# fcogidi/X3D-tf

Hardware: AMD Instinct MI355X
Metric: clips/sec (fwd+bwd) X3D-M 16x224^2; depthwise HBM GB/s (higher is better)
Workload: dtype bf16

## Files before the change

### x3d-tf_amd/csrc/pw_gemm_bf16.h

```cpp
#pragma once
#include <stdlib.h>

#include "pw_gemm.h"

typedef __attribute__((ext_vector_type(4))) short s16x4;
typedef __attribute__((ext_vector_type(8))) short s16x8;

#define PWB_BN 128
#define PWB_KCH 64
#define PWB_XP (PWB_BN + 32)
#define PWB_OP (PWB_BN + 4)

template <typename H, int VEC, int MT, int PRO, int EPI, int STRIDED, int OVEC, bool RAG = false>
__global__ __launch_bounds__(256) void pw_gemm_bf16_kernel(const PwGemmArgs a) {
  typedef typename HV<H>::x8 hx8; typedef typename HV<H>::x4 hx4; typedef typename HV<H>::x2 hx2;
  extern __shared__ __attribute__((aligned(16))) unsigned char smem_raw[];
  typedef H T;
  constexpr int BM = MT * 32, BN = PWB_BN, XP = PWB_XP, OP = PWB_OP, KCH = PWB_KCH;
  constexpr bool HAS_SUMS = (EPI == EPI_STATS) || (EPI == X3D_EPI_SWISH_BWD);
  constexpr bool BSTORE = (OVEC == 8);
  typedef __attribute__((ext_vector_type(4))) unsigned int u32x4_;
  constexpr int VPR = BN / VEC;
  constexpr int NSV = (KCH * VPR + 255) / 256;
  constexpr int ROWS_PT = BM / 16;
  constexpr int SLAB = (MT <= 2) ? MT : 1, NSLAB = MT / SLAB, ROWS_SL = 2 * SLAB;
  const int Kp = a.KC;
  const int WP = Kp + 8;
  constexpr size_t XO_BYTES = ((size_t)KCH * XP * 2 > (size_t)SLAB * 32 * OP * 4) ? (size_t)KCH * XP * 2 : (size_t)SLAB * 32 * OP * 4;
  H* Xs = (H*)smem_raw;
  float* Os = (float*)smem_raw;
  H* Ws = (H*)(smem_raw + XO_BYTES);
  float* Cs = (float*)(smem_raw + XO_BYTES + (size_t)BM * (a.KC + 8) * 2);

  const int tid = threadIdx.x, lane = tid & 63, wid = tid >> 6;
  const int r = lane & 31, half = lane >> 5;
  const int m0 = blockIdx.y * BM;
  const int tiles_per_n = (int)((a.P + BN - 1) / BN);
  const int total_tiles = tiles_per_n * a.N;
  const int tile_begin = blockIdx.x * a.tiles_per_block;
  const int tile_end = min(tile_begin + a.tiles_per_block, total_tiles);
  const int nkc = (Kp + KCH - 1) / KCH;

  if (a.wp) {
    const hx8* src = (const hx8*)((const H*)a.wp + (long long)m0 * WP);
    const int nvec = BM * WP / 8;
    const int lim = max(0, min(BM, a.wp_rows - m0)) * WP / 8;
    hx8 zero;
#pragma unroll
    for (int e = 0; e < 8; e++) zero[e] = (H)0.f;
#pragma unroll 4
    for (int i = tid; i < nvec; i += 256) ((hx8*)Ws)[i] = i < lim ? src[i] : zero;
  } else {
    const int wv = a.wvec;
    if (a.wsk == 1) {
      const int kv = Kp / wv;
      for (int i = tid; i < BM * kv; i += 256) {
        const int m = i / kv, k = (i - m * kv) * wv;
        const int gm = m0 + m;
        const float* src = a.w + (long long)gm * a.wsm + k;
        H* dst = &Ws[m * WP + k];
        for (int e = 0; e < wv; e += 1) dst[e] = (H)0.f;
        if (gm < a.M && k < a.K) {
          if (wv == 4) { const f32x4 v = *(const f32x4*)src; dst[0] = (H)v[0]; dst[1] = (H)v[1]; dst[2] = (H)v[2]; dst[3] = (H)v[3]; }
          else if (wv == 2) { const float2 v = *(const float2*)src; dst[0] = (H)v.x; dst[1] = (H)v.y; }
          else dst[0] = (H)src[0];
        }
      }
    } else {
      const int mv = BM / wv;
      for (int i = tid; i < Kp * mv; i += 256) {
        const int k = i / mv, m = (i - k * mv) * wv;
        const int gm = m0 + m;
        const float* src = a.w + (long long)k * a.wsk + gm;
        float v[4] = {0.f, 0.f, 0.f, 0.f};
        if (k < a.K) {
          if (wv == 4 && gm + 3 < a.M) { const f32x4 t = *(const f32x4*)src; v[0] = t[0]; v[1] = t[1]; v[2] = t[2]; v[3] = t[3]; }
          else for (int e = 0; e < wv; e++) if (gm + e < a.M) v[e] = src[e];
        }
        for (int e = 0; e < wv; e++) Ws[(m + e) * WP + k] = (H)v[e];
      }
    }
  }

  constexpr bool AFF = (PRO == PRO_AFFINE) || (PRO == PRO_AFFST);
  constexpr int CSW = AFF ? 2 : 4;
  const bool use_cs = AFF || a.K < 320;
  auto fill_coef = [&](int n) {
    if (!use_cs) return;
    if constexpr (PRO != PRO_NONE) {
      for (int k = tid; k < Kp; k += 256) {
        f32x4 c = {0.f, 0.f, 0.f, 0.f};
        if (k < a.K) {
          if constexpr (AFF) {
            const float g = a.gate ? a.gate[(long long)n * a.K + k] : 1.0f;
            c[0] = a.coef[k * 2] * g;
            c[1] = a.coef[k * 2 + 1] * g;
          } else if constexpr (PRO == PRO_TAIL) {
            c[0] = a.coef[k * 2]; c[1] = a.coef2 ? a.coef2[k * 2] : 1.0f;
            c[2] = a.coef[k * 2 + 1] + (a.coef2 ? a.coef2[k * 2 + 1] : 0.f);
          } else {
            c[0] = a.coef[k * 4]; c[1] = a.coef[k * 4 + 1]; c[2] = a.coef[k * 4 + 2];
          }
        }
        if constexpr (CSW == 2) *(float2*)&Cs[k * 2] = make_float2(c[0], c[1]);
        else *(f32x4*)&Cs[k * 4] = c;
      }
    }
  };
  if (tile_begin < tile_end) fill_coef(tile_begin / tiles_per_n);

  constexpr bool TWO = (PRO == PRO_BNBWD) || (PRO == PRO_TAIL);
  hx8 xr[NSV], yr[(TWO || STRIDED) ? NSV : 1];
  float xs1[(VEC == 1) ? NSV : 1], ys1[(VEC == 1 && TWO) ? NSV : 1];
  auto issue_loads = [&](int tile, int kc_idx) {
    const int n = tile / tiles_per_n;
    const long long p0 = (long long)(tile - n * tiles_per_n) * BN;
    const int k0 = kc_idx * KCH;
    const int kc = min(KCH, Kp - k0);
#pragma unroll
    for (int i = 0; i < NSV; i++) {
      const int v = tid + i * 256;
      const int k = v / VPR, pv = v - k * VPR;
      const int gk = k0 + k;
      const long long p = p0 + (long long)pv * VEC;
      const bool ok = (k < kc) && (gk < a.K) && (p < a.P);
      if constexpr (VEC == 8) {
        hx8 z;
#pragma unroll
        for (int e = 0; e < 8; e++) z[e] = (H)0.f;
        xr[i] = z;
        if constexpr (TWO) yr[i] = z;
        if constexpr (STRIDED) yr[i] = z;
        if (ok) {
          if constexpr (STRIDED) {
            strided_gather16<STRIDED>((const T*)a.x + ((long long)n * a.K + gk) * a.Pin, p, a.H, a.W, a.Ho, a.Wo, xr[i], yr[i],
                                      RAG ? (int)min((long long)8, a.P - p) : 8);
          } else {
            const long long o = ((long long)n * a.K + k0 + (tid >> 4)) * a.Pin + p0 + (tid & 15) * 8 + (long long)i * 16 * a.Pin;
            const long long left = RAG ? a.P - p : 8;
            if (left >= 8) {
              xr[i] = *(const hx8*)((const T*)a.x + o);
              if constexpr (TWO) yr[i] = *(const hx8*)((const T*)a.x2 + o);
            } else {
              xr[i] = load8_ragged<T, hx8>((const T*)a.x + o, (int)left);
              if constexpr (TWO) yr[i] = load8_ragged<T, hx8>((const T*)a.x2 + o, (int)left);
            }
          }
        }
      } else {
        xs1[i] = 0.f;
        if constexpr (TWO) ys1[i] = 0.f;
        if (ok) {
          long long src = p;
          if constexpr (STRIDED) {
            const int hw = a.Ho * a.Wo;
            const int t = (int)p / hw;
            const int rem = (int)p - t * hw;
            const int ho = rem / a.Wo, wo = rem - ho * a.Wo;
            src = ((long long)t * a.H + (long long)ho * a.stride) * a.W + (long long)wo * a.stride;
          }
          const long long o = ((long long)n * a.K + gk) * a.Pin + src;
          xs1[i] = to_f<T>(((const T*)a.x)[o]);
          if constexpr (TWO) ys1[i] = to_f<T>(((const T*)a.x2)[o]);
        }
      }
    }
  };
  auto commit = [&](int tile, int kc_idx) {
    const int n = tile / tiles_per_n;
    const int k0 = kc_idx * KCH;
    const int kc = min(KCH, Kp - k0);
#pragma unroll
    for (int i = 0; i < NSV; i++) {
      const int v = tid + i * 256;
      const int k = v / VPR, pv = v - k * VPR;
      if (k >= kc) continue;
      const int gk = k0 + k;
      H* dst = &Xs[k * XP + pv * VEC];
      if constexpr (PRO == PRO_NONE) {
        if constexpr (VEC == 8 && STRIDED) {
          hx8 o;
#pragma unroll
          for (int e = 0; e < 4; e++) { o[e] = xr[i][2 * e]; o[4 + e] = yr[i][2 * e]; }
          *(hx8*)dst = o;
        } else if constexpr (VEC == 8) *(hx8*)dst = xr[i];
        else dst[0] = (H)xs1[i];
      } else {
        float val[VEC];
        if constexpr (VEC == 8) {
#pragma unroll
          for (int e = 0; e < 8; e++) val[e] = (float)xr[i][e];
        } else {
          val[0] = xs1[i];
        }
        f32x4 cf;
        if (use_cs) {
          if constexpr (CSW == 2) { const float2 t2 = *(const float2*)&Cs[gk * 2]; cf[0] = t2.x; cf[1] = t2.y; cf[2] = 0.f; cf[3] = 0.f; }
          else cf = *(const f32x4*)&Cs[gk * 4];
        } else {
          const bool inb = gk < a.K;
          cf[3] = 0.f;
          if constexpr (AFF) {
            const float g = (inb && a.gate) ? a.gate[(long long)n * a.K + gk] : 1.0f;
            cf[0] = inb ? a.coef[gk * 2] * g : 0.f; cf[1] = inb ? a.coef[gk * 2 + 1] * g : 0.f; cf[2] = 0.f;
          } else if constexpr (PRO == PRO_TAIL) {
            cf[0] = inb ? a.coef[gk * 2] : 0.f; cf[1] = (inb && a.coef2) ? a.coef2[gk * 2] : (inb ? 1.0f : 0.f);
            cf[2] = inb ? a.coef[gk * 2 + 1] + (a.coef2 ? a.coef2[gk * 2 + 1] : 0.f) : 0.f;
          } else {
            cf[0] = inb ? a.coef[gk * 4] : 0.f; cf[1] = inb ? a.coef[gk * 4 + 1] : 0.f; cf[2] = inb ? a.coef[gk * 4 + 2] : 0.f;
          }
        }
        if constexpr (AFF) {
#pragma unroll
          for (int e = 0; e < VEC; e++) val[e] = cf[0] * val[e] + cf[1];
          act_vec<VEC>(val, a.act);
        } else {
#pragma unroll
          for (int e = 0; e < VEC; e++) {
            const float y2 = (VEC == 8) ? (float)yr[i][e] : ys1[i];
            val[e] = cf[0] * val[e] + cf[1] * y2 + cf[2];
            if constexpr (PRO == PRO_TAIL) val[e] = fmaxf(val[e], 0.f);
          }
        }
        VecIO<H, VEC>::store(dst, val);
        if constexpr (PRO == PRO_TAIL || PRO == PRO_AFFST) {
          const int n_ = tile / tiles_per_n;
          const long long p_ = (long long)(tile - n_ * tiles_per_n) * BN + (long long)pv * VEC;
          if (blockIdx.y == 0 && gk < a.K && p_ < a.P) {
            T* yd = (T*)a.ystore + ((long long)n_ * a.K + gk) * a.Pin + p_;
            if constexpr (VEC == 8) {
              if (!RAG || a.P - p_ >= 8) VecIO<T, 8>::store(yd, val);
              else for (int e = 0; e < (int)(a.P - p_); e++) yd[e] = from_f<T>(val[e]);
            } else {
              yd[0] = from_f<T>(val[0]);
            }
          }
        }
      }
    }
  };

  float st1[HAS_SUMS ? ROWS_PT : 1], st2[HAS_SUMS ? ROWS_PT : 1];
  if constexpr (HAS_SUMS) {
#pragma unroll
    for (int i = 0; i < ROWS_PT; i++) { st1[i] = 0.f; st2[i] = 0.f; }
  }

  const int g16 = lane >> 4, q = (lane & 15) >> 2, pp = lane & 3;
  const int tr_col = wid * 32 + 16 * (g16 & 1) + 4 * pp;
  const int tr_row = 8 * (g16 >> 1) + q;
  typedef s16x4 __attribute__((address_space(3))) * lds_s16x4_ptr;

  f32x16 acc[MT];
  if (tile_begin < tile_end) issue_loads(tile_begin, 0);
  if constexpr (BSTORE) {
    __amdgpu_buffer_rsrc_t r0 = __builtin_amdgcn_make_buffer_rsrc((T*)a.y, 0, 0, 0x00020000);
    u32x4_ z0 = {0u, 0u, 0u, 0u};
#pragma unroll
    for (int i = 0; i < ROWS_PT; i++) __builtin_amdgcn_raw_buffer_store_b128(z0, r0, 0x80000000u, 0, 0);
  }

  auto flush_sums = [&](int n) {
    if constexpr (HAS_SUMS) {
#pragma unroll
      for (int i = 0; i < ROWS_PT; i++) {
        float s1 = st1[i], s2 = st2[i];
        s1 = row16_sum(s1);
        s2 = row16_sum(s2);
        const int m = m0 + (tid >> 4) + 16 * i;
        if ((tid & 15) == 0 && m < a.M) {
          if constexpr (EPI == EPI_STATS) {
            if (a.stats) {
              double* sp = stats_replica(a.stats, a.M, blockIdx.x);
              atomic_add_d(&sp[m * 2], (double)s1);
              atomic_add_d(&sp[m * 2 + 1], (double)s2);
            }
          } else {
            double* d = a.nc_sums + ((long long)n * a.M + m) * 2;
            atomic_add_d(d, (double)s1);
            atomic_add_d(d + 1, (double)s2);
          }
        }
        st1[i] = 0.f;
        st2[i] = 0.f;
      }
    }
  };

  float bna_s[EPI == EPI_BNADD ? ROWS_PT : 1], bna_t[EPI == EPI_BNADD ? ROWS_PT : 1], bna_g[EPI == EPI_BNADD ? ROWS_PT : 1];
  if constexpr (EPI == EPI_BNADD) {
#pragma unroll
    for (int i = 0; i < ROWS_PT; i++) {
      const int m = m0 + (tid >> 4) + 16 * i;
      bnadd_coef(a, m, m < a.M, bna_s[i], bna_t[i], bna_g[i]);
    }
  }

  int n_prev = tile_begin < tile_end ? tile_begin / tiles_per_n : 0;
  for (int tile = tile_begin; tile < tile_end; ++tile) {
    const int n = tile / tiles_per_n;
    const long long p0 = (long long)(tile - n * tiles_per_n) * BN;
    if constexpr (EPI == X3D_EPI_SWISH_BWD) {
      if (n != n_prev) flush_sums(n_prev);
    }
    if constexpr (AFF) {
      if (n != n_prev && a.gate) fill_coef(n);
    }
    n_prev = n;
#pragma unroll
    for (int s = 0; s < MT; s++)
#pragma unroll
      for (int j = 0; j < 16; j++) acc[s][j] = 0.f;

    for (int kc_idx = 0; kc_idx < nkc; ++kc_idx) {
      const int k0 = kc_idx * KCH;
      const int kc = min(KCH, Kp - k0);
      __syncthreads();
      commit(tile, kc_idx);
      __syncthreads();
      if (kc_idx + 1 < nkc) issue_loads(tile, kc_idx + 1);
      else if (tile + 1 < tile_end) issue_loads(tile + 1, 0);
      for (int kk = 0; kk < kc; kk += 16) {
        const s16x4 b0 = __builtin_amdgcn_ds_read_tr16_b64_v4i16((lds_s16x4_ptr)(&Xs[(kk + tr_row) * XP + tr_col]));
        const s16x4 b1 = __builtin_amdgcn_ds_read_tr16_b64_v4i16((lds_s16x4_ptr)(&Xs[(kk + tr_row + 4) * XP + tr_col]));
        const s16x8 bs = {b0[0], b0[1], b0[2], b0[3], b1[0], b1[1], b1[2], b1[3]};
        const hx8 bfrag = __builtin_bit_cast(hx8, bs);
#pragma unroll
        for (int s = 0; s < MT; s++) {
          const hx8 afrag = *(const hx8*)&Ws[(s * 32 + r) * WP + k0 + kk + 8 * half];
          acc[s] = mfma16<H>(afrag, bfrag, acc[s]);
        }
      }
    }

    const int oc = (tid & 15) * 8;
    __amdgpu_buffer_rsrc_t yrsrc;
    if constexpr (BSTORE)
      yrsrc = __builtin_amdgcn_make_buffer_rsrc((T*)a.y + (long long)n * a.M * a.P, 0, (int)((long long)a.M * a.P * 2), 0x00020000);
    constexpr bool BNA_ = (EPI == EPI_BNADD);
    constexpr bool EPL8 = (OVEC == 8) && (EPI == X3D_EPI_ADD || EPI == X3D_EPI_SWISH_BWD || BNA_);
    constexpr bool EPL4 = (OVEC == 8) && (EPI == X3D_EPI_ADD_STRIDED);
    hx8 epl8[EPL8 ? ROWS_PT : 1];
    hx4 epl4[EPL4 ? ROWS_PT : 1];
    const int egv = !EPL4 ? 0 : ((a.eW & 7) == 0 ? 8 : ((a.eW & 3) == 0 ? 4 : ((a.eW & 1) == 0 ? 2 : 0)));
    const bool epl4_vec = egv != 0;
    constexpr bool SWB_ = (EPI == X3D_EPI_SWISH_BWD);
    float esb[(SWB_ || BNA_) ? ROWS_PT : 1], etb[(SWB_ || BNA_) ? ROWS_PT : 1], egt[(SWB_ || BNA_) ? ROWS_PT : 1];
    if constexpr (BNA_) {
#pragma unroll
      for (int i = 0; i < ROWS_PT; i++) { esb[i] = bna_s[i]; etb[i] = bna_t[i]; egt[i] = bna_g[i]; }
    }
    if constexpr (SWB_) {
#pragma unroll
      for (int i = 0; i < ROWS_PT; i++) {
        const int m = m0 + (tid >> 4) + 16 * i;
        const bool ok = m < a.M;
        esb[i] = ok ? a.b_ss[m * 2] : 0.f;
        etb[i] = ok ? a.b_ss[m * 2 + 1] : 0.f;
        egt[i] = (ok && a.egate) ? a.egate[(long long)n * a.M + m] : 1.0f;
      }
    }
    if constexpr (EPL8 || EPL4) {
#pragma unroll
      for (int i = 0; i < ROWS_PT; i++) {
        const int m = m0 + (tid >> 4) + 16 * i;
        const long long p = p0 + oc;
        if constexpr (EPL8) {
#pragma unroll
          for (int e = 0; e < 8; e++) epl8[i][e] = (H)0.f;
          if (m < a.M && p < a.P && (!BNA_ || a.add)) {
            const long long o = ((long long)n * a.M + m) * a.P + p;
            const T* src = (const T*)(EPI == X3D_EPI_SWISH_BWD ? a.braw : a.add) + o;
            if (!RAG || a.P - p >= 8) epl8[i] = *(const hx8*)src;
            else epl8[i] = load8_ragged<T, hx8>(src, (int)(a.P - p));
          }
        } else {
#pragma unroll
          for (int e = 0; e < 4; e++) epl4[i][e] = (H)0.f;
          if (epl4_vec && m < a.M && p < a.P) {
            const int hw = a.eH * a.eW;
            const int Hh = (a.eH + 1) >> 1, Wh = (a.eW + 1) >> 1;
            const int T_ = (int)a.P / hw;
            const T* abase = (const T*)a.add + ((long long)n * a.M + m) * T_ * Hh * Wh;
            if (egv == 8) {
              const int t = (int)p / hw;
              const int rem = (int)p - t * hw;
              const int h = rem / a.eW, w = rem - h * a.eW;
              if ((h & 1) == 0) epl4[i] = *(const hx4*)(abase + ((long long)t * Hh + (h >> 1)) * Wh + (w >> 1));
            } else if (egv == 4) {
#pragma unroll
              for (int gq = 0; gq < 2; gq++) {
                const int pe = (int)p + 4 * gq;
                if (RAG && pe >= (int)a.P) continue;
                const int t = pe / hw;
                const int rem = pe - t * hw;
                const int h = rem / a.eW, w = rem - h * a.eW;
                if ((h & 1) == 0) {
                  const hx2 v2 = *(const hx2*)(abase + ((long long)t * Hh + (h >> 1)) * Wh + (w >> 1));
                  epl4[i][2 * gq] = v2[0]; epl4[i][2 * gq + 1] = v2[1];
                }
              }
            } else {
#pragma unroll
              for (int gq = 0; gq < 4; gq++) {
                const int pe = (int)p + 2 * gq;
                if (RAG && pe >= (int)a.P) continue;
                const int t = pe / hw;
                const int rem = pe - t * hw;
                const int h = rem / a.eW, w = rem - h * a.eW;
                if ((h & 1) == 0) epl4[i][gq] = abase[((long long)t * Hh + (h >> 1)) * Wh + (w >> 1)];
              }
            }
          }
        }
      }
    }
#pragma unroll
    for (int sl = 0; sl < NSLAB; sl++) {
    __syncthreads();
#pragma unroll
    for (int s = 0; s < SLAB; s++)
#pragma unroll
      for (int j = 0; j < 16; j++)
        Os[(s * 32 + (j & 3) + 8 * (j >> 2) + 4 * half) * OP + wid * 32 + r] = acc[sl * SLAB + s][j];
    __syncthreads();
#pragma unroll
    for (int ii = 0; ii < ROWS_SL; ii++) {
      const int i = sl * ROWS_SL + ii;
      const int row = (tid >> 4) + 16 * ii;
      const int m = m0 + sl * SLAB * 32 + row;
      const long long p = p0 + oc;
      const bool rvalid = (m < a.M) && (p < a.P);
      if constexpr (!BSTORE) { if (!rvalid) continue; }
      float val[8];
      {
        const f32x4 v0 = *(const f32x4*)&Os[row * OP + oc], v1 = *(const f32x4*)&Os[row * OP + oc + 4];
#pragma unroll
        for (int e = 0; e < 4; e++) { val[e] = v0[e]; val[4 + e] = v1[e]; }
      }
      const long long o = ((long long)n * a.M + m) * a.P + p;
      const int nvalid = (OVEC == 8 && !RAG) ? 8 : (int)min((long long)8, a.P - p);
      if constexpr (EPI == X3D_EPI_ADD) {
        if constexpr (OVEC == 8) {
#pragma unroll
          for (int e = 0; e < 8; e++) val[e] += (float)epl8[i][e];
        } else {
          for (int e = 0; e < nvalid; e++) val[e] += to_f<T>(((const T*)a.add)[o + e]);
        }
      } else if constexpr (BNA_) {
        float ad[8];
        if constexpr (OVEC == 8) {
#pragma unroll
          for (int e = 0; e < 8; e++) ad[e] = (float)epl8[i][e];
        } else {
          for (int e = 0; e < 8; e++) ad[e] = (e < nvalid && a.add) ? to_f<T>(((const T*)a.add)[o + e]) : 0.f;
        }
        const float lo = a.eact == X3D_ACT_RELU ? 0.f : -__builtin_inff();
#pragma unroll
        for (int e = 0; e < 8; e++) val[e] = fmaxf(esb[i] * val[e] + etb[i] + egt[i] * ad[e], lo);
      } else if constexpr (EPI == X3D_EPI_ADD_STRIDED) {
        const int hw = a.eH * a.eW;
        const int Hh = (a.eH + 1) >> 1, Wh = (a.eW + 1) >> 1;
        const int T_ = (int)a.P / hw;
        if (epl4_vec) {
          if constexpr (EPL4) {
#pragma unroll
            for (int e = 0; e < 4; e++) val[2 * e] += (float)epl4[i][e];
          }
        } else if (m < a.M)
        for (int e = 0; e < nvalid; e++) {
          const int pe = (int)p + e;
          const int t = pe / hw;
          const int rem = pe - t * hw;
          const int h = rem / a.eW, w = rem - h * a.eW;
          if (((h | w) & 1) == 0) {
            const long long oa = ((((long long)n * a.M + m) * T_ + t) * Hh + (h >> 1)) * Wh + (w >> 1);
            val[e] += to_f<T>(((const T*)a.add)[oa]);
          }
        }
      } else if constexpr (EPI == X3D_EPI_SWISH_BWD) {
        float b[8];
        if constexpr (OVEC == 8) {
#pragma unroll
          for (int e = 0; e < 8; e++) b[e] = (float)epl8[i][e];
        } else {
          for (int e = 0; e < 8; e++) b[e] = (e < nvalid) ? to_f<T>(((const T*)a.braw)[o + e]) : 0.f;
        }
        const SwishCoef sc_ = swish_coef(esb[i], etb[i], egt[i]);
#pragma unroll
        for (int e = 0; e < 8; e++) {
          float xh_, d_;
          swish_bwd_(sc_, b[e], xh_, d_);
          const float dv = val[e] * d_;
          val[e] = dv;
          if (e < nvalid && rvalid) {
            st1[i] += dv;
            st2[i] += dv * b[e];
          }
        }
      }
      if constexpr (EPI == EPI_STATS) {
#pragma unroll
        for (int e = 0; e < 8; e++) {
          if (e < nvalid && rvalid) {
            st1[i] += val[e];
            st2[i] += val[e] * val[e];
          }
        }
      }
      if constexpr (BSTORE) {
        hx8 ov;
#pragma unroll
        for (int e = 0; e < 8; e++) ov[e] = (H)val[e];
        const unsigned off = (rvalid && (!RAG || nvalid == 8)) ? (unsigned)(((long long)m * a.P + p) * 2) : 0x80000000u;
        __builtin_amdgcn_raw_buffer_store_b128(__builtin_bit_cast(u32x4_, ov), yrsrc, off, 0, 0);
        if constexpr (RAG) {
          if (rvalid && nvalid < 8) store8_ragged<T, hx8>((T*)a.y + o, ov, nvalid);
        }
      } else if constexpr (OVEC == 8) {
        if (!RAG || nvalid == 8) VecIO<T, 8>::store((T*)a.y + o, val);
        else {
          for (int e = 0; e < nvalid; e++) ((T*)a.y)[o + e] = from_f<T>(val[e]);
        }
      } else {
        for (int e = 0; e < nvalid; e++) ((T*)a.y)[o + e] = from_f<T>(val[e]);
      }
    }
    }
  }

  if (tile_begin < tile_end) flush_sums(n_prev);
}

static inline size_t pw_bf16_lds_bytes(int mt, int K) {
  const int slab = mt <= 2 ? mt : 1;
  const size_t xb = (size_t)PWB_KCH * PWB_XP * 2, ob = (size_t)slab * 32 * PWB_OP * 4;
  return (xb > ob ? xb : ob) + (size_t)mt * 32 * (((K + 15) & ~15) + 8) * 2 + (K < 320 ? (size_t)((K + 15) & ~15) * 16 : (size_t)((K + 15) & ~15) * 8);
}

static inline int pw_bf16_pick_mt(int M, int K) {
  const int mt = ceil_div(M, 32);
#ifdef X3D_EXPERIMENTS
  const char* map = getenv("X3D_PW_MTMAP");
#else
  const char* map = nullptr;
#endif
  if (map) {
    for (const char* q = map; *q;) {
      const int key = atoi(q);
      const char* c = strchr(q, ':');
      if (!c) break;
      const int val = atoi(c + 1);
      if (key == mt && (val == 1 || val == 2 || val == 3 || val == 4 || val == 7) && pw_bf16_lds_bytes(val, K) <= 160 * 1024) return val;
      const char* n = strchr(c, ',');
      if (!n) break;
      q = n + 1;
    }
  }
  if (mt <= 1 || K >= 320) return 1;
  if (mt == 3 && pw_bf16_lds_bytes(3, K) <= 80 * 1024) return 3;
  return 2;
}

template <typename H, int VEC, int MT, int PRO, int EPI, int STRIDED, int OVEC, bool RAG = false>
static int pw_bf16_launch_cfg(PwGemmArgs& a, hipStream_t st) {
  if constexpr (!RAG && VEC == 8 && OVEC == 8) {
    if (a.P % 8 != 0) return pw_bf16_launch_cfg<H, VEC, MT, PRO, EPI, STRIDED, OVEC, true>(a, st);
  }
  constexpr int BM = MT * 32, BN = PWB_BN;
  a.KC = (a.K + 15) & ~15;
  const size_t lds = pw_bf16_lds_bytes(MT, a.K);
  X3D_REQUIRE(lds <= 160 * 1024, "pw_gemm_bf16: K = %d needs %zu B of LDS", a.K, lds);
  const int gy = ceil_div(a.M, BM);
  const long long total_tiles = ceil_div_ll(a.P, BN) * a.N;
  X3D_REQUIRE(total_tiles < (1ll << 31), "pw_gemm_bf16: too many tiles");
  X3D_REQUIRE((long long)a.M * a.P * 2 < (1ll << 31), "pw_gemm_bf16: one sample's output exceeds the 2 GB buffer-store window");
  X3D_DESCRIBE("pw_gemm_bf16_kernel<%s, %d, %d, %d, %d, %d, %d, %d>", HV<H>::name, VEC, MT, PRO, EPI, STRIDED, OVEC, (int)RAG);
  auto kern = pw_gemm_bf16_kernel<H, VEC, MT, PRO, EPI, STRIDED, OVEC, RAG>;
  if (lds > 48 * 1024) {
    static bool attr_set = false;
    if (!attr_set) {
      (void)hipFuncSetAttribute((const void*)kern, hipFuncAttributeMaxDynamicSharedMemorySize, 160 * 1024);
      attr_set = true;
    }
  }
  static size_t occ_lds[8];
  static int occ_slots[8], occ_n = 0;
  int slots = 0;
  for (int i = 0; i < occ_n; i++) if (occ_lds[i] == lds) slots = occ_slots[i];
  if (slots == 0) {
    int nb = 0, dev = 0, cus = 256;
    hipDeviceProp_t prop;
    if (hipGetDevice(&dev) == hipSuccess && hipGetDeviceProperties(&prop, dev) == hipSuccess) cus = prop.multiProcessorCount;
    if (hipOccupancyMaxActiveBlocksPerMultiprocessor(&nb, kern, 256, lds) != hipSuccess || nb < 1) nb = 1;
    slots = nb * cus;
    if (occ_n < 8) { occ_lds[occ_n] = lds; occ_slots[occ_n] = slots; occ_n++; }
  }
  long long gx_target = slots / gy;
  if (gx_target < 1) gx_target = 1;
  int tpb = (int)ceil_div_ll(total_tiles, gx_target);
  int tpb_min = a.K >= 192 ? 4 : (a.K >= 96 ? 2 : 1);
  tpb_min = x3d_env_int("X3D_PW_TPBMIN", tpb_min);
  if (tpb < tpb_min) tpb = tpb_min;
  a.tiles_per_block = tpb;
  const long long gx = ceil_div_ll(total_tiles, tpb);
  {
    const int contig = (a.wsk == 1) ? a.K : a.M;
    int wv = 4;
    while (wv > 1 && ((contig % wv) != 0 || ((uintptr_t)a.w % (wv * 4)) != 0)) wv >>= 1;
    if (a.wsk != 1 && (BM % wv) != 0) wv = 1;
    a.wvec = wv;
  }
  hipLaunchKernelGGL(kern, dim3((unsigned)gx, gy), dim3(256), lds, st, a);
  X3D_LAUNCH_CHECK("pw_gemm_bf16");
  return X3D_OK;
}

template <typename H, int VEC, int PRO, int EPI, int STRIDED, int OVEC>
static int pw_bf16_launch_tile(PwGemmArgs& a, hipStream_t st) {
  int mt = pw_bf16_pick_mt(a.M, a.K);
  if constexpr (VEC == 1) mt = mt > 2 ? 2 : mt;
  switch (mt) {
    case 7: if constexpr (VEC != 1) return pw_bf16_launch_cfg<H, VEC, 7, PRO, EPI, STRIDED, OVEC>(a, st);
    case 4: if constexpr (VEC != 1) return pw_bf16_launch_cfg<H, VEC, 4, PRO, EPI, STRIDED, OVEC>(a, st);
    case 3: if constexpr (VEC != 1) return pw_bf16_launch_cfg<H, VEC, 3, PRO, EPI, STRIDED, OVEC>(a, st);
    case 2: return pw_bf16_launch_cfg<H, VEC, 2, PRO, EPI, STRIDED, OVEC>(a, st);
    default: return pw_bf16_launch_cfg<H, VEC, 1, PRO, EPI, STRIDED, OVEC>(a, st);
  }
}

template <typename H, int PRO, int EPI>
static int pw_bf16_launch_vec(PwGemmArgs& a, int vec, int ovec, hipStream_t st) {
  if (a.stride > 1) {
    if constexpr (PRO == PRO_NONE && EPI == EPI_STATS) {
      const int gv = (a.stride == 2 && vec >= 1 && ovec >= 8) ? strided_gather_gv(a.W, a.Wo, a.P, a.x) : 0;
      if (gv == 4) return pw_bf16_launch_tile<H, 8, PRO, EPI, 4, 8>(a, st);
      if (gv == 2) return pw_bf16_launch_tile<H, 8, PRO, EPI, 2, 8>(a, st);
      if (gv == 1) return pw_bf16_launch_tile<H, 8, PRO, EPI, 1, 8>(a, st);
      if (ovec >= 8 && a.P % 8 == 0) return pw_bf16_launch_tile<H, 1, PRO, EPI, 1, 8>(a, st);
      return pw_bf16_launch_tile<H, 1, PRO, EPI, 1, 1>(a, st);
    } else {
      x3d_set_error("pw: strided gather only in forward");
      return X3D_ERR_INVALID;
    }
  }
  if (vec >= 8 && ovec >= 8) return pw_bf16_launch_tile<H, 8, PRO, EPI, 0, 8>(a, st);
  return pw_bf16_launch_tile<H, 1, PRO, EPI, 0, 1>(a, st);
}
```

Measured before the change: 3256.

## Use raw buffer loads/stores with OOB masking for PRO_AFFST pointwise GEMM prologue

For the non-ragged, non-strided PRO_AFFST bf16 pointwise GEMM path, the per-element bounds-checked global loads and side stores are replaced with 128-bit raw buffer loads and stores. Out-of-range rows and columns are masked by setting the offset to an out-of-bounds value or shrinking the buffer extent, which removes per-element branches and index math. The loop also issues the next tile's loads unconditionally and adds dummy OOB stores, likely to keep wait-count/scheduling uniform. A WIDE fallback variant handles inputs too large for the 32-bit buffer offset. Occupancy queries now use the variant with the extra registers, at the cost of added code complexity and different register pressure.

```diff
diff --git a/x3d-tf_amd/csrc/pw_gemm_bf16.h b/x3d-tf_amd/csrc/pw_gemm_bf16.h
--- a/x3d-tf_amd/csrc/pw_gemm_bf16.h
+++ b/x3d-tf_amd/csrc/pw_gemm_bf16.h
@@ -11,7 +11,7 @@
 #define PWB_XP (PWB_BN + 32)
 #define PWB_OP (PWB_BN + 4)
 
-template <typename H, int VEC, int MT, int PRO, int EPI, int STRIDED, int OVEC, bool RAG = false>
+template <typename H, int VEC, int MT, int PRO, int EPI, int STRIDED, int OVEC, bool RAG = false, bool WIDE = false>
 __global__ __launch_bounds__(256) void pw_gemm_bf16_kernel(const PwGemmArgs a) {
   typedef typename HV<H>::x8 hx8; typedef typename HV<H>::x4 hx4; typedef typename HV<H>::x2 hx2;
   extern __shared__ __attribute__((aligned(16))) unsigned char smem_raw[];
@@ -19,6 +19,8 @@
   constexpr int BM = MT * 32, BN = PWB_BN, XP = PWB_XP, OP = PWB_OP, KCH = PWB_KCH;
   constexpr bool HAS_SUMS = (EPI == EPI_STATS) || (EPI == X3D_EPI_SWISH_BWD);
   constexpr bool BSTORE = (OVEC == 8);
+  constexpr bool BUFL = (VEC == 8) && (OVEC == 8) && !RAG && !WIDE && (PRO == PRO_AFFST) && (STRIDED == 0) && (MT <= 3);
+  constexpr unsigned OOB = 0x80000000u;
   typedef __attribute__((ext_vector_type(4))) unsigned int u32x4_;
   constexpr int VPR = BN / VEC;
   constexpr int NSV = (KCH * VPR + 255) / 256;
@@ -40,6 +42,7 @@
   const int tile_begin = blockIdx.x * a.tiles_per_block;
   const int tile_end = min(tile_begin + a.tiles_per_block, total_tiles);
   const int nkc = (Kp + KCH - 1) / KCH;
+  const unsigned vrow = (unsigned)(((long long)(tid >> 4) * a.Pin + (tid & 15) * 8) * 2);
 
   if (a.wp) {
     const hx8* src = (const hx8*)((const H*)a.wp + (long long)m0 * WP);
@@ -117,6 +120,22 @@
     const long long p0 = (long long)(tile - n * tiles_per_n) * BN;
     const int k0 = kc_idx * KCH;
     const int kc = min(KCH, Kp - k0);
+    if constexpr (BUFL) {
+      const int rows = tile < tile_end ? a.K - k0 : 0;
+      const long long pleft = a.P - p0;
+      const bool colok = (tid & 15) * 8 < pleft;
+      const long long base = ((long long)n * a.K + k0) * a.Pin + p0;
+#pragma unroll
+      for (int i = 0; i < NSV; i++) {
+        const int ri = min(rows - 16 * i, 16);
+        const int bytes = ri > 0 ? (int)(((long long)(ri - 1) * a.Pin + pleft) * 2) : 0;
+        const unsigned vo = (colok && (tid >> 4) < ri) ? vrow : OOB;
+        const long long o = base + (long long)i * 16 * a.Pin;
+        const __amdgpu_buffer_rsrc_t rx = __builtin_amdgcn_make_buffer_rsrc((T*)a.x + o, 0, bytes, 0x00020000);
+        xr[i] = __builtin_bit_cast(hx8, __builtin_amdgcn_raw_buffer_load_b128(rx, vo, 0, 0));
+      }
+      return;
+    }
 #pragma unroll
     for (int i = 0; i < NSV; i++) {
       const int v = tid + i * 256;
@@ -170,11 +189,17 @@
     const int n = tile / tiles_per_n;
     const int k0 = kc_idx * KCH;
     const int kc = min(KCH, Kp - k0);
+    constexpr bool SIDE = BUFL;
+    const int s_rows = SIDE ? a.K - k0 : 0;
+    const long long s_pleft = SIDE ? a.P - (long long)(tile - n * tiles_per_n) * BN : 0;
+    const long long s_base = SIDE ? ((long long)n * a.K + k0) * a.Pin + (long long)(tile - n * tiles_per_n) * BN : 0;
 #pragma unroll
     for (int i = 0; i < NSV; i++) {
       const int v = tid + i * 256;
       const int k = v / VPR, pv = v - k * VPR;
-      if (k >= kc) continue;
+      u32x4_ sv = {0u, 0u, 0u, 0u};
+      unsigned svo = OOB;
+      if (BUFL ? (16 * i < kc) : (k < kc)) {
       const int gk = k0 + k;
       H* dst = &Xs[k * XP + pv * VEC];
       if constexpr (PRO == PRO_NONE) {
@@ -223,7 +248,13 @@
           }
         }
         VecIO<H, VEC>::store(dst, val);
-        if constexpr (PRO == PRO_TAIL || PRO == PRO_AFFST) {
+        if constexpr (SIDE) {
+          hx8 ov;
+#pragma unroll
+          for (int e = 0; e < 8; e++) ov[e] = (H)val[e];
+          sv = __builtin_bit_cast(u32x4_, ov);
+          svo = ((tid & 15) * 8 < s_pleft && (tid >> 4) < s_rows - 16 * i) ? vrow : OOB;
+        } else if constexpr (PRO == PRO_TAIL || PRO == PRO_AFFST) {
           const int n_ = tile / tiles_per_n;
           const long long p_ = (long long)(tile - n_ * tiles_per_n) * BN + (long long)pv * VEC;
           if (blockIdx.y == 0 && gk < a.K && p_ < a.P) {
@@ -237,6 +268,13 @@
           }
         }
       }
+      }
+      if constexpr (SIDE) {
+        const int ri = min(s_rows - 16 * i, 16);
+        const int bytes = (ri > 0 && blockIdx.y == 0) ? (int)(((long long)(ri - 1) * a.Pin + s_pleft) * 2) : 0;
+        const __amdgpu_buffer_rsrc_t rs = __builtin_amdgcn_make_buffer_rsrc((T*)a.ystore + s_base + (long long)i * 16 * a.Pin, 0, bytes, 0x00020000);
+        __builtin_amdgcn_raw_buffer_store_b128(sv, rs, svo, 0, 0);
+      }
     }
   };
 
@@ -257,7 +295,7 @@
     __amdgpu_buffer_rsrc_t r0 = __builtin_amdgcn_make_buffer_rsrc((T*)a.y, 0, 0, 0x00020000);
     u32x4_ z0 = {0u, 0u, 0u, 0u};
 #pragma unroll
-    for (int i = 0; i < ROWS_PT; i++) __builtin_amdgcn_raw_buffer_store_b128(z0, r0, 0x80000000u, 0, 0);
+    for (int i = 0; i < ROWS_PT; i++) __builtin_amdgcn_raw_buffer_store_b128(z0, r0, 0x80000000u + (BUFL ? 16u * i : 0u), 0, 0);
   }
 
   auto flush_sums = [&](int n) {
@@ -318,8 +356,13 @@
       __syncthreads();
       commit(tile, kc_idx);
       __syncthreads();
-      if (kc_idx + 1 < nkc) issue_loads(tile, kc_idx + 1);
-      else if (tile + 1 < tile_end) issue_loads(tile + 1, 0);
+      if constexpr (BUFL) {
+        const bool last = kc_idx + 1 == nkc;
+        issue_loads(last ? tile + 1 : tile, last ? 0 : kc_idx + 1);
+      } else {
+        if (kc_idx + 1 < nkc) issue_loads(tile, kc_idx + 1);
+        else if (tile + 1 < tile_end) issue_loads(tile + 1, 0);
+      }
       for (int kk = 0; kk < kc; kk += 16) {
         const s16x4 b0 = __builtin_amdgcn_ds_read_tr16_b64_v4i16((lds_s16x4_ptr)(&Xs[(kk + tr_row) * XP + tr_col]));
         const s16x4 b1 = __builtin_amdgcn_ds_read_tr16_b64_v4i16((lds_s16x4_ptr)(&Xs[(kk + tr_row + 4) * XP + tr_col]));
@@ -330,6 +373,12 @@
           const hx8 afrag = *(const hx8*)&Ws[(s * 32 + r) * WP + k0 + kk + 8 * half];
           acc[s] = mfma16<H>(afrag, bfrag, acc[s]);
         }
+      }
+      if constexpr (BUFL) {
+        __amdgpu_buffer_rsrc_t r0 = __builtin_amdgcn_make_buffer_rsrc((T*)a.y, 0, 0, 0x00020000);
+        u32x4_ z0 = {0u, 0u, 0u, 0u};
+#pragma unroll
+        for (int i = 0; i < ROWS_PT; i++) __builtin_amdgcn_raw_buffer_store_b128(z0, r0, OOB + 16u * i, 0, 0);
       }
     }
 
@@ -562,10 +611,13 @@
   return 2;
 }
 
-template <typename H, int VEC, int MT, int PRO, int EPI, int STRIDED, int OVEC, bool RAG = false>
+template <typename H, int VEC, int MT, int PRO, int EPI, int STRIDED, int OVEC, bool RAG = false, bool WIDE = false>
 static int pw_bf16_launch_cfg(PwGemmArgs& a, hipStream_t st) {
-  if constexpr (!RAG && VEC == 8 && OVEC == 8) {
+  if constexpr (!RAG && !WIDE && VEC == 8 && OVEC == 8) {
     if (a.P % 8 != 0) return pw_bf16_launch_cfg<H, VEC, MT, PRO, EPI, STRIDED, OVEC, true>(a, st);
+    if constexpr (PRO == PRO_AFFST && STRIDED == 0 && MT <= 3) {
+      if (a.Pin >= (1ll << 26)) return pw_bf16_launch_cfg<H, VEC, MT, PRO, EPI, STRIDED, OVEC, false, true>(a, st);
+    }
   }
   constexpr int BM = MT * 32, BN = PWB_BN;
   a.KC = (a.K + 15) & ~15;
@@ -576,11 +628,15 @@
   X3D_REQUIRE(total_tiles < (1ll << 31), "pw_gemm_bf16: too many tiles");
   X3D_REQUIRE((long long)a.M * a.P * 2 < (1ll << 31), "pw_gemm_bf16: one sample's output exceeds the 2 GB buffer-store window");
   X3D_DESCRIBE("pw_gemm_bf16_kernel<%s, %d, %d, %d, %d, %d, %d, %d>", HV<H>::name, VEC, MT, PRO, EPI, STRIDED, OVEC, (int)RAG);
-  auto kern = pw_gemm_bf16_kernel<H, VEC, MT, PRO, EPI, STRIDED, OVEC, RAG>;
+  auto kern = pw_gemm_bf16_kernel<H, VEC, MT, PRO, EPI, STRIDED, OVEC, RAG, WIDE>;
+  auto occ_kern = pw_gemm_bf16_kernel<H, VEC, MT, PRO, EPI, STRIDED, OVEC, RAG,
+                                      WIDE || (!RAG && VEC == 8 && OVEC == 8 && STRIDED == 0 && PRO == PRO_AFFST && MT <= 3)>;
   if (lds > 48 * 1024) {
     static bool attr_set = false;
     if (!attr_set) {
       (void)hipFuncSetAttribute((const void*)kern, hipFuncAttributeMaxDynamicSharedMemorySize, 160 * 1024);
+      if ((const void*)occ_kern != (const void*)kern)
+        (void)hipFuncSetAttribute((const void*)occ_kern, hipFuncAttributeMaxDynamicSharedMemorySize, 160 * 1024);
       attr_set = true;
     }
   }
@@ -592,7 +648,7 @@
     int nb = 0, dev = 0, cus = 256;
     hipDeviceProp_t prop;
     if (hipGetDevice(&dev) == hipSuccess && hipGetDeviceProperties(&prop, dev) == hipSuccess) cus = prop.multiProcessorCount;
-    if (hipOccupancyMaxActiveBlocksPerMultiprocessor(&nb, kern, 256, lds) != hipSuccess || nb < 1) nb = 1;
+    if (hipOccupancyMaxActiveBlocksPerMultiprocessor(&nb, occ_kern, 256, lds) != hipSuccess || nb < 1) nb = 1;
     slots = nb * cus;
     if (occ_n < 8) { occ_lds[occ_n] = lds; occ_slots[occ_n] = slots; occ_n++; }
   }
```

Result: no change. 3277 (median of 6 runs) (+0.6%).
